# WHOIGit/ifcb_classifier

Hardware: AMD Instinct MI355X
Metric: train images/sec, inception_v3 299^2 IFCB ROIs (higher is better)
Workload: dtype bf16; 1 GPU; inception_v3 100-class bf16 TRAIN, batch 256 per GPU, synthetic u8 ROIs h,w~U{32..299} resized on-GPU to 299x299 (BASELINE.json configs[1]); global_batch=256, parallelism=dp1, program_lanes=4, IFCBK_LANES=4, weight_gradient_lanes=1, optimizer=adam lr=1e-3, loss=CE + 0.4*CE_aux, input_pipeline=preprocess then step on one stream

## Files before the change

ifcb_classifier_amd/csrc/conv_common.h:

```cpp
#pragma once
#include "common.h"

namespace {

struct ConvArgs {
    const void* x;
    const void* w;
    void* y;
    float* part;
    const float* ep_scale;
    const float* ep_shift;
    const void* ep_res;
    int ep_ldr, ep_relu;
    const void* bs_raw;
    const float *bs_mean, *bs_invstd, *bs_scale, *bs_shift;
    int bs_ld;
    const void* pad_;
    unsigned xbytes, wbytes;
    int H, W, C, ldx;
    int K, R, S;
    int P, Q, ldy;
    int ostr_h, ostr_w, base_h, base_w, ish, isw;
    int M, Kg;
    int accumulate;
    int seg_n, seg_end[4], seg_ld[4], seg_aff[4];
    void* seg_y[4];
    int PQ;
    int tilesN;
    int wKg, wSfull, w_rbase, w_sbase;
    int oH, oW, o_a, o_b;
    fastdiv_t fPQ, fQ;
    int tr;
    fastdiv_t fP;
    int dbg;
};

typedef const __attribute__((address_space(1))) void* gptr_t;
typedef __attribute__((address_space(3))) void* lptr_t;

template <class T> struct Mma;
template <> struct Mma<bf16_t> {
    typedef bf16x8_t frag_t;
    __device__ static __forceinline__ void run(const frag_t& a, const frag_t& b, f32x4_t& c) {
        c = __builtin_amdgcn_mfma_f32_16x16x32_bf16(a, b, c, 0, 0, 0);
    }
    __device__ static __forceinline__ void pack4(bf16_t* p, const f32x4_t& v) {
        uint2 u;
        u.x = pack2bf(v[0], v[1]);
        u.y = pack2bf(v[2], v[3]);
        *reinterpret_cast<uint2*>(p) = u;
    }
};
template <> struct Mma<float> {
    typedef f32x4_t frag_t;
    __device__ static __forceinline__ void run(const frag_t& a, const frag_t& b, f32x4_t& c) {
#pragma unroll
        for (int j = 0; j < 4; ++j) c = __builtin_amdgcn_mfma_f32_16x16x4f32(a[j], b[j], c, 0, 0, 0);
    }
    __device__ static __forceinline__ void pack4(float* p, const f32x4_t& v) { *reinterpret_cast<f32x4_t*>(p) = v; }
};

__device__ __forceinline__ void lds_dma16(__amdgpu_buffer_rsrc_t rs, lptr_t dst, unsigned voff, int soff) {
    __builtin_amdgcn_raw_ptr_buffer_load_lds(rs, dst, 16, voff, soff, 0, 0);
}

template <int N>
__device__ __forceinline__ void wait_vmcnt() {
    asm volatile("s_waitcnt vmcnt(%0)" ::"n"(N) : "memory");
}


template <class T, int BM, int BN, int NTHREADS, int MODE>
__device__ __forceinline__ void conv_epilogue_store(const ConvArgs& a, T* sC, float* sRed, const int t, const int lane, const int wave,
                                                    const int m0, const int n0, const int mtile) {
    constexpr bool BSTAT = MODE == 3;
    constexpr int ES = (int)sizeof(T);
    constexpr int CE = 16 / ES;
    constexpr int NW = NTHREADS / 64;
    constexpr int CPR = BN / CE;
    constexpr int CPRP = CPR <= 4 ? 4 : CPR <= 8 ? 8 : CPR <= 16 ? 16 : 32;
    constexpr int LDC = BN + CE;
    {
        constexpr int RPP = NTHREADS / CPRP;
        const int cc = t & (CPRP - 1);
        const int r0 = t / CPRP;
        const bool cvalid = (cc < CPR) && (n0 + cc * CE < a.K);
        typedef float f32x2_t __attribute__((ext_vector_type(2)));
        f32x2_t s1p[CE / 2], s2p[CE / 2];
#pragma unroll
        for (int j = 0; j < CE / 2; ++j) s1p[j] = s2p[j] = f32x2_t{0.f, 0.f};
        if (cvalid) {
            const int nn = n0 + cc * CE;
            float bmu[CE], bis[CE], bsc[CE], bsh[CE];
            if (BSTAT) {
#pragma unroll
                for (int j = 0; j < CE; ++j) {
                    bmu[j] = a.bs_mean[nn + j];
                    bis[j] = a.bs_invstd[nn + j];
                    bsc[j] = a.bs_scale[nn + j];
                    bsh[j] = a.bs_shift[nn + j];
                }
            }
            float sc[CE], sh[CE];
            if (a.ep_scale) {
#pragma unroll
                for (int j = 0; j < CE; ++j) {
                    sc[j] = a.ep_scale[nn + j];
                    sh[j] = a.ep_shift[nn + j];
                }
            }
            T* segbase = (T*)a.y + nn;
            int segld = a.ldy;
            bool seg_aff = true;
            if (MODE == 4) {
                int si = 0;
#pragma unroll
                for (int q = 0; q < 3; ++q)
                    if (q + 1 < a.seg_n && nn >= a.seg_end[q]) si = q + 1;
                segbase = (T*)a.seg_y[si] + (nn - (si ? a.seg_end[si - 1] : 0));
// ... 128 lines not shown
```

ifcb_classifier_amd/csrc/conv_igemm.hip:

```cpp
#include "conv_common.h"
#include <stdlib.h>

namespace {

template <class T, int NT, int WM, int NSTAGE, int MODE>
__global__ __launch_bounds__(128 * WM) void conv_igemm(ConvArgs a) {
    constexpr bool STRIDED = MODE == 1;
    constexpr int ES = (int)sizeof(T);
    constexpr int CE = 16 / ES;
    constexpr int BK = 128 / ES;
    typedef typename Mma<T>::frag_t frag_t;
    constexpr int NW = 2 * WM;
    constexpr int NTHREADS = 64 * NW;
    constexpr int BM = 64 * WM;
    constexpr int BN = 32 * NT;
    constexpr int JB = (NT * 4 + NW - 1) / NW;
    constexpr int G = 4 + JB;
    constexpr int D = NSTAGE - 1;
    constexpr int LDC = BN + CE;
    constexpr int STAGE = (BM + BN) * BK;
    constexpr int STAGE_BYTES = NSTAGE * STAGE * ES;
    constexpr int CT_BYTES = BM * LDC * ES + NW * BN * 2 * 4;
    constexpr int MAIN_BYTES = STAGE_BYTES > CT_BYTES ? STAGE_BYTES : CT_BYTES;
    constexpr int DUMMY_BYTES = (JB * NW > NT * 4) ? 1024 : 0;
    __shared__ __attribute__((aligned(16))) unsigned char smem[MAIN_BYTES + DUMMY_BYTES];
    T* sStage = reinterpret_cast<T*>(smem);
    T* sC = reinterpret_cast<T*>(smem);
    float* sRed = reinterpret_cast<float*>(smem + BM * LDC * ES);
    T* sDummy = reinterpret_cast<T*>(smem + MAIN_BYTES);

    const int t = threadIdx.x;
    const int lane = t & 63;
    const int wave = __builtin_amdgcn_readfirstlane(t >> 6);
    const int wm = wave >> 1, wn = wave & 1;
    const int bid = (int)xcd_remap(blockIdx.x, gridDim.x);
    const int mtile = bid / a.tilesN, ntile = bid - mtile * a.tilesN;
    const int m0 = mtile * BM, n0 = ntile * BN;

    const __amdgpu_buffer_rsrc_t rsA = __builtin_amdgcn_make_buffer_rsrc((void*)a.x, 0, a.xbytes, 0x00020000);
    const __amdgpu_buffer_rsrc_t rsB = __builtin_amdgcn_make_buffer_rsrc((void*)a.w, 0, a.wbytes, 0x00020000);
    constexpr unsigned OOB = 0x80000000u;
    const int lrow8 = lane >> 3;
    const int csrc = (lane & 7) ^ lrow8;
    int off0[4], bh[4], bw[4];
#pragma unroll
    for (int j = 0; j < 4; ++j) {
        int m = m0 + (wave * 4 + j) * 8 + lrow8;
        bool rv = m < a.M;
        int mm = rv ? m : 0;
        int n = (int)fdiv((uint32_t)mm, a.fPQ);
        int rem = mm - n * a.PQ;
        int p = (int)fdiv((uint32_t)rem, a.fQ);
        int q = rem - p * a.Q;
        bh[j] = rv ? p * a.ostr_h + a.base_h : -(1 << 24);
        bw[j] = q * a.ostr_w + a.base_w;
        off0[j] = STRIDED ? n * a.H * a.W * a.ldx : ((n * a.H + bh[j]) * a.W + bw[j]) * a.ldx;
    }
    int kc, kr, ks, tapoff;
    {
        kc = csrc * CE;
        kr = 0;
        ks = 0;
        while (kc >= a.C) {
            kc -= a.C;
            if (++ks == a.S) { ks = 0; ++kr; }
        }
        tapoff = (kr * a.W + ks) * a.ldx + kc;
    }
    int wk = MODE == 2 ? ((a.w_rbase + 2 * kr) * a.wSfull + a.w_sbase + 2 * ks) * a.C + kc : 0;
    unsigned woff[JB];
    bool gvalid[JB];
#pragma unroll
    for (int j = 0; j < JB; ++j) {
        int grp = j * NW + wave;
        gvalid[j] = grp < NT * 4;
        int n = n0 + grp * 8 + lrow8;
        woff[j] = (gvalid[j] && n < a.K) ? (MODE == 2 ? (unsigned)(n * a.wKg) : (unsigned)(n * a.Kg + csrc * CE)) * (unsigned)ES : OOB;
    }
    const int nk = (a.Kg + BK - 1) / BK;
    const int hmask = (1 << a.ish) - 1, wmask = (1 << a.isw) - 1;
    const int rowstep = a.W * a.ldx, colwrap = a.S * a.ldx;
    const int wrowskip = MODE == 2 ? (2 * a.wSfull - 2 * a.S) * a.C : 0;

    const bool plain = (MODE == 0 || MODE == 3 || MODE == 4) && a.R == 1 && a.S == 1 && a.base_h == 0 && a.base_w == 0;
    unsigned va[4];
#pragma unroll
    for (int j = 0; j < 4; ++j) va[j] = bh[j] >= 0 ? (unsigned)(off0[j] + csrc * CE) * (unsigned)ES : OOB;
    const bool ktail_ok = (nk - 1) * BK + csrc * CE < a.Kg;

#define ISSUE_TILE(kt, stage)                                                                              \
    {                                                                                                      \
        T* dstA = sStage + (stage) * STAGE;                                                                \
        T* dstB = dstA + BM * BK;                                                                          \
        if (plain) {                                                                                       \
            const bool cut = (kt) == nk - 1 && !ktail_ok;                                                  \
            _Pragma("unroll") for (int j = 0; j < 4; ++j)                                                  \
                lds_dma16(rsA, (lptr_t)(dstA + (wave * 4 + j) * 8 * BK), cut ? OOB : va[j], (kt) * 128);   \
        } else {                                                                                           \
            const bool kvalid = kr < a.R;                                                                  \
            _Pragma("unroll") for (int j = 0; j < 4; ++j) {                                                \
                int hr = bh[j] + kr, wr = bw[j] + ks;                                                      \
                unsigned voff;                                                                             \
                if (STRIDED) {                                                                             \
                    bool v = kvalid && hr >= 0 && wr >= 0 && ((hr & hmask) == 0) && ((wr & wmask) == 0);   \
                    int hi = hr >> a.ish, wi = wr >> a.isw;                                                \
                    v = v && hi < a.H && wi < a.W;                                                         \
                    voff = v ? (unsigned)(off0[j] + (hi * a.W + wi) * a.ldx + kc) * (unsigned)ES : OOB;    \
                } else {                                                                                   \
                    bool v = kvalid && (unsigned)hr < (unsigned)a.H && (unsigned)wr < (unsigned)a.W;       \
                    voff = v ? (unsigned)(off0[j] + tapoff) * (unsigned)ES : OOB;                          \
                }                                                                                          \
                __builtin_amdgcn_raw_ptr_buffer_load_lds(rsA, (lptr_t)(dstA + (wave * 4 + j) * 8 * BK), 16, voff, 0, 0, 0); \
            }                                                                                              \
        }                                                                                                  \
        if (MODE == 2) {                                                                                   \
            const bool kv2 = ((kt) * BK + csrc * CE) < a.Kg;                                               \
            _Pragma("unroll") for (int j = 0; j < JB; ++j) {                                               \
                unsigned voff = (kv2 && woff[j] != OOB) ? woff[j] + (unsigned)wk * (unsigned)ES : OOB;     \
// ... 5 lines not shown
            _Pragma("unroll") for (int j = 0; j < JB; ++j) {                                               \
                T* dst = gvalid[j] ? dstB + (j * NW + wave) * 8 * BK : sDummy;                             \
                lds_dma16(rsB, (lptr_t)dst, woff[j], (kt) * 128);                                          \
            }                                                                                              \
        }                                                                                                  \
        if (!plain) {                                                                                      \
            kc += BK;                                                                                      \
            tapoff += BK;                                                                                  \
            if (MODE == 2) wk += BK;                                                                       \
            while (kc >= a.C) {                                                                            \
                kc -= a.C;                                                                                 \
                tapoff += a.ldx - a.C;                                                                     \
                if (MODE == 2) wk += a.C;                       \
                if (++ks == a.S) { ks = 0; ++kr; tapoff += rowstep - colwrap; if (MODE == 2) wk += wrowskip; } \
            }                                                                                              \
        }                                                                                                  \
    }

    f32x4_t acc[NT][4];
#pragma unroll
    for (int i = 0; i < NT; ++i)
#pragma unroll
        for (int j = 0; j < 4; ++j) acc[i][j] = f32x4_t{0.f, 0.f, 0.f, 0.f};

#pragma unroll
    for (int d = 0; d < D; ++d)
        if (d < nk) ISSUE_TILE(d, d)

    const int frow = lane & 15, fchunk = lane >> 4;
    const T* fA[2];
    const T* fB[2];
#pragma unroll
    for (int kk = 0; kk < 2; ++kk) {
        const int ph = ((kk * 4 + fchunk) ^ (frow & 7)) * CE;
        fA[kk] = sStage + (wm * 64 + frow) * BK + ph;
        fB[kk] = sStage + BM * BK + (wn * (NT * 16) + frow) * BK + ph;
    }
    int stage = 0;
    int istage = D % NSTAGE;
    for (int kt = 0; kt < nk; ++kt) {
        const int newer = nk - 1 - kt < D - 1 ? nk - 1 - kt : D - 1;
        if (D >= 3 && newer >= 2) wait_vmcnt<2 * G>();
        else if (D >= 2 && newer >= 1) wait_vmcnt<G>();
        else wait_vmcnt<0>();
        __builtin_amdgcn_s_barrier();
        if (kt + D < nk) ISSUE_TILE(kt + D, istage)
        const int soff = stage * STAGE;
#pragma unroll
        for (int kk = 0; kk < 2; ++kk) {
            frag_t fa[4], fb[NT];
            const T* pa = fA[kk] + soff;
            const T* pb = fB[kk] + soff;
#pragma unroll
            for (int mt = 0; mt < 4; ++mt) fa[mt] = *reinterpret_cast<const frag_t*>(pa + mt * 16 * BK);
#pragma unroll
            for (int nt = 0; nt < NT; ++nt) fb[nt] = *reinterpret_cast<const frag_t*>(pb + nt * 16 * BK);
#pragma unroll
            for (int nt = 0; nt < NT; ++nt)
#pragma unroll
                for (int mt = 0; mt < 4; ++mt)
                    Mma<T>::run(fb[nt], fa[mt], acc[nt][mt]);
        }
        stage = stage + 1 == NSTAGE ? 0 : stage + 1;
        istage = istage + 1 == NSTAGE ? 0 : istage + 1;
    }
#undef ISSUE_TILE
    __syncthreads();

    {
        const int g = lane >> 4;
#pragma unroll
        for (int nt = 0; nt < NT; ++nt)
#pragma unroll
            for (int mt = 0; mt < 4; ++mt) {
                int m = wm * 64 + mt * 16 + frow;
                int n = wn * (NT * 16) + nt * 16 + 4 * g;
                Mma<T>::pack4(sC + m * LDC + n, acc[nt][mt]);
            }
    }
    __syncthreads();
    conv_epilogue_store<T, BM, BN, NTHREADS, MODE>(a, sC, sRed, t, lane, wave, m0, n0, mtile);
}

template <int NT>
__global__ __launch_bounds__(512) void conv_ws(ConvArgs a, int total_tiles) {
    typedef bf16_t T;
    constexpr int ES = 2, CE = 8, BK = 64, BM = 128, BN = 32 * NT, NSTAGE = 3;
    constexpr int STAGE = (BM + BN) * BK;
    constexpr int G = 4 + NT;
    __shared__ __attribute__((aligned(16))) unsigned char smem[NSTAGE * STAGE * ES];
    T* sStage = reinterpret_cast<T*>(smem);
    const int t = threadIdx.x, lane = t & 63;
    const int wave = __builtin_amdgcn_readfirstlane(t >> 6);
    const int b0 = (int)xcd_remap(blockIdx.x, gridDim.x);
    const int ngrid = (int)gridDim.x;
    const int ntl = (total_tiles - b0 + ngrid - 1) / ngrid;
    const int nk = (a.Kg + BK - 1) / BK;
    const int total_steps = ntl * nk;

    if (wave >= 4) {
        const int p = wave - 4;
        const __amdgpu_buffer_rsrc_t rsA = __builtin_amdgcn_make_buffer_rsrc((void*)a.x, 0, a.xbytes, 0x00020000);
        const __amdgpu_buffer_rsrc_t rsB = __builtin_amdgcn_make_buffer_rsrc((void*)a.w, 0, a.wbytes, 0x00020000);
        constexpr unsigned OOB = 0x80000000u;
        const int lrow8 = lane >> 3;
        const int csrc = (lane & 7) ^ lrow8;
        const bool plain = a.R == 1 && a.S == 1 && a.base_h == 0 && a.base_w == 0;
        const bool ktail_ok = (nk - 1) * BK + csrc * CE < a.Kg;
        const int rowstep = a.W * a.ldx, colwrap = a.S * a.ldx;
        int off0[4], bh[4], bw[4];
        unsigned va[4], woff[NT];
        int kc = 0, kr = 0, ks = 0, tapoff = 0, kt_issue = 0, r_issue = 0;
#define WS_SETUP_TILE(tile)                                                                                   \
        {                                                                                                     \
            const int mtile_ = (tile) / a.tilesN, ntile_ = (tile) - mtile_ * a.tilesN;                        \
            const int m0_ = mtile_ * BM, n0_ = ntile_ * BN;                                                   \
            _Pragma("unroll") for (int j = 0; j < 4; ++j) {                                                   \
                int m = m0_ + (p * 4 + j) * 8 + lrow8;                                                        \
                bool rv = m < a.M;                                                                            \
                int mm = rv ? m : 0;                                                                          \
                int n = (int)fdiv((uint32_t)mm, a.fPQ);                                                       \
                int rem = mm - n * a.PQ;                                                                      \
                int pp = (int)fdiv((uint32_t)rem, a.fQ);                                                      \
                int q = rem - pp * a.Q;                                                                       \
                bh[j] = rv ? pp * a.ostr_h + a.base_h : -(1 << 24);                                           \
                bw[j] = q * a.ostr_w + a.base_w;                                                              \
                off0[j] = ((n * a.H + bh[j]) * a.W + bw[j]) * a.ldx;                                          \
                va[j] = bh[j] >= 0 ? (unsigned)(off0[j] + csrc * CE) * (unsigned)ES : OOB;                    \
            }                                                                                                 \
            _Pragma("unroll") for (int j = 0; j < NT; ++j) {                                                  \
                int n = n0_ + (j * 4 + p) * 8 + lrow8;                                                        \
                woff[j] = n < a.K ? (unsigned)(n * a.Kg + csrc * CE) * (unsigned)ES : OOB;                    \
            }                                                                                                 \
            kc = csrc * CE; kr = 0; ks = 0;                                                                   \
            while (kc >= a.C) { kc -= a.C; if (++ks == a.S) { ks = 0; ++kr; } }                               \
            tapoff = (kr * a.W + ks) * a.ldx + kc;                                                            \
        }
#define WS_ISSUE(stage)                                                                                       \
        {                                                                                                     \
            if (kt_issue == 0) WS_SETUP_TILE(b0 + r_issue * ngrid)                                            \
            T* dstA = sStage + (stage) * STAGE;                                                               \
            T* dstB = dstA + BM * BK;                                                                         \
            if (plain) {                                                                                      \
                const bool cut = kt_issue == nk - 1 && !ktail_ok;                                             \
                _Pragma("unroll") for (int j = 0; j < 4; ++j)                                                 \
                    lds_dma16(rsA, (lptr_t)(dstA + (p * 4 + j) * 8 * BK), cut ? OOB : va[j], kt_issue * 128); \
            } else {                                                                                          \
                const bool kvalid = kr < a.R;                                                                 \
                _Pragma("unroll") for (int j = 0; j < 4; ++j) {                                               \
                    int hr = bh[j] + kr, wr = bw[j] + ks;                                                     \
                    bool v = kvalid && (unsigned)hr < (unsigned)a.H && (unsigned)wr < (unsigned)a.W;          \
                    unsigned voff = v ? (unsigned)(off0[j] + tapoff) * (unsigned)ES : OOB;                    \
                    __builtin_amdgcn_raw_ptr_buffer_load_lds(rsA, (lptr_t)(dstA + (p * 4 + j) * 8 * BK), 16, voff, 0, 0, 0); \
                }                                                                                             \
                kc += BK;                                                                                     \
                tapoff += BK;                                                                                 \
                while (kc >= a.C) {                                                                           \
                    kc -= a.C;                                                                                \
                    tapoff += a.ldx - a.C;                                                                    \
                    if (++ks == a.S) { ks = 0; ++kr; tapoff += rowstep - colwrap; }                           \
                }                                                                                             \
            }                                                                                                 \
            _Pragma("unroll") for (int j = 0; j < NT; ++j)                                                    \
                lds_dma16(rsB, (lptr_t)(dstB + (j * 4 + p) * 8 * BK), woff[j], kt_issue * 128);               \
            if (++kt_issue == nk) { kt_issue = 0; ++r_issue; }                                                \
        }
// ... 74 lines not shown
                    sc[j] = nv ? a.ep_scale[ncol + nt * 16 + j] : 0.f;
                    sh[j] = nv ? a.ep_shift[ncol + nt * 16 + j] : 0.f;
                }
            }
            f32x2_t s1[2] = {f32x2_t{0.f, 0.f}, f32x2_t{0.f, 0.f}}, s2[2] = {f32x2_t{0.f, 0.f}, f32x2_t{0.f, 0.f}};
#pragma unroll
            for (int mt = 0; mt < 4; ++mt) {
                f32x4_t v = acc[nt][mt];
                if (a.ep_scale) {
#pragma unroll
                    for (int j = 0; j < 4; ++j) {
                        v[j] = bf2f(f2bf(v[j])) * sc[j] + sh[j];
                        if (a.ep_relu) v[j] = fmaxf(v[j], 0.f);
                    }
                }
                uint2 u;
                u.x = pack2bf(v[0], v[1]);
                u.y = pack2bf(v[2], v[3]);
                if (mv[mt] && nv) *reinterpret_cast<uint2*>(row[mt] + nt * 16) = u;
                const f32x2_t lo = {__uint_as_float(u.x << 16), __uint_as_float(u.x & 0xffff0000u)};
                const f32x2_t hi = {__uint_as_float(u.y << 16), __uint_as_float(u.y & 0xffff0000u)};
                s1[0] += lo; s1[1] += hi;
                s2[0] += lo * lo; s2[1] += hi * hi;
            }
            if (a.part) {
#pragma unroll
                for (int off = 1; off < 16; off <<= 1)
#pragma unroll
                    for (int h = 0; h < 2; ++h)
#pragma unroll
                        for (int j = 0; j < 2; ++j) {
                            s1[h][j] += __shfl_xor(s1[h][j], off);
                            s2[h][j] += __shfl_xor(s2[h][j], off);
                        }
                if (frow == 0 && nv) {
                    float* prow = a.part + ((size_t)(mtile * 2 + wm) * 2) * a.K + ncol + nt * 16;
#pragma unroll
                    for (int j = 0; j < 4; ++j) {
                        prow[j] = s1[j >> 1][j & 1];
                        prow[a.K + j] = s2[j >> 1][j & 1];
                    }
                }
            }
        }
    }
}

int pick_nt(int K, int maxnt) {
    static int force = -1;
    if (force < 0) { const char* e = getenv("IFCBK_CONV_NT"); force = e ? atoi(e) : 0; }
    if (force > 0 && force <= maxnt) return force;
    int best = 1;
    long bestc = -1;
    for (int nt = 1; nt <= maxnt; ++nt) {
        int bn = 32 * nt;
        long c = (long)cdiv(K, bn) * (bn + 48);
        if (bestc < 0 || c < bestc || (c == bestc && nt > best)) { bestc = c; best = nt; }
    }
    return best;
}

int check_desc(ifcbk_ctx* ctx, const ifcbk_conv_desc* d, bool dgrad = false) {
    if (!d) IFCBK_FAIL(ctx, IFCBK_EINVAL, "conv: null desc");
    if (d->dtype != IFCBK_BF16 && d->dtype != IFCBK_F32) IFCBK_FAIL(ctx, IFCBK_EUNSUPPORTED, "conv: dtype must be bf16 or f32");
    const int ce = dtype_chunk(d->dtype), es = dtype_esize(d->dtype);
    if (d->C % ce || d->K % ce || d->ldx % ce || d->ldy % ce || d->C <= 0 || d->K <= 0)
        IFCBK_FAIL(ctx, IFCBK_EINVAL, "conv: C=%d K=%d ldx=%d ldy=%d must be positive multiples of %d", d->C, d->K, d->ldx, d->ldy, ce);
    if (d->stride_h < 1 || d->stride_w < 1 || (dgrad && (d->stride_h > 2 || d->stride_w > 2)))
        IFCBK_FAIL(ctx, IFCBK_EINVAL, "conv: stride must be >= 1 (1 or 2 for the input gradient)");
    int P = (d->H + 2 * d->pad_h - d->R) / d->stride_h + 1, Q = (d->W + 2 * d->pad_w - d->S) / d->stride_w + 1;
    if (P != d->P || Q != d->Q) IFCBK_FAIL(ctx, IFCBK_EINVAL, "conv: P,Q=%d,%d inconsistent (expect %d,%d)", d->P, d->Q, P, Q);
    if ((int64_t)d->N * d->P * d->Q * d->ldy * es >= (1ll << 31) || (int64_t)d->N * d->H * d->W * d->ldx * es >= (1ll << 31))
        IFCBK_FAIL(ctx, IFCBK_EINVAL, "conv: a tensor exceeds the 2 GiB buffer-descriptor window");
    return 0;
}

int pick_wm(int M, int K) {
    static int force = -1;
    if (force < 0) { const char* e = getenv("IFCBK_CONV_WM"); force = e ? atoi(e) : 0; }
    (void)M; (void)K;
    return force == 4 ? 4 : 2;
}

template <class T, int NT, int WM, int NSTAGE>
void launch(const ConvArgs& a, hipStream_t st) {
    int tilesM = cdiv(a.M, 64 * WM);
    dim3 grid((unsigned)(tilesM * a.tilesN)), block(128 * WM);
    if (a.seg_n) hipLaunchKernelGGL((conv_igemm<T, NT, WM, NSTAGE, 4>), grid, block, 0, st, a);
    else if (a.bs_raw) hipLaunchKernelGGL((conv_igemm<T, NT, WM, NSTAGE, 3>), grid, block, 0, st, a);
    else if (a.wKg) hipLaunchKernelGGL((conv_igemm<T, NT, WM, NSTAGE, 2>), grid, block, 0, st, a);
    else if (a.ish | a.isw) hipLaunchKernelGGL((conv_igemm<T, NT, WM, NSTAGE, 1>), grid, block, 0, st, a);
    else hipLaunchKernelGGL((conv_igemm<T, NT, WM, NSTAGE, 0>), grid, block, 0, st, a);
}

int ws_min_steps() {
    static int v = -1;
    if (v < 0) { const char* e = getenv("IFCBK_CONV_WS"); v = e ? atoi(e) : 4; }
    return v;
}
int num_cus();
int ws_max_tiles() {
    static int v = -1;
    if (v < 0) { const char* e = getenv("IFCBK_CONV_WS_TILES"); v = e ? atoi(e) : 2 * num_cus(); }
    return v;
}
bool ws_shape_ok(int dtype, int M, int K, int Kg) {
    const int ms = ws_min_steps();
    if (ms <= 0 || dtype != IFCBK_BF16 || pick_wm(M, K) != 2 || cdiv(Kg, 64) < ms) return false;
    const int nt = pick_nt(K, 6);
    return (int64_t)cdiv(M, 128) * cdiv(K, 32 * nt) <= ws_max_tiles();
}
int num_cus() {
    static int n = 0;
    if (!n) {
        int dev = 0;
        hipDeviceProp_t pr;
        if (hipGetDevice(&dev) == hipSuccess && hipGetDeviceProperties(&pr, dev) == hipSuccess) n = pr.multiProcessorCount;
        if (n <= 0) n = 256;
    }
    return n;
}

template <int NT>
void launch_ws(const ConvArgs& a, hipStream_t st) {
    const int total = cdiv(a.M, 128) * a.tilesN;
    const int grid = total < num_cus() ? total : num_cus();
    hipLaunchKernelGGL((conv_ws<NT>), dim3((unsigned)grid), dim3(512), 0, st, a, total);
}

bool big_ok(const ConvArgs& a) { return !a.wKg && !(a.ish | a.isw); }
bool pp3_ok(const ConvArgs& a) {
    return big_ok(a) && !a.seg_n && !a.bs_raw && !a.accumulate && !a.ep_res && (a.ep_scale == nullptr || a.part == nullptr);
}

int run(ifcbk_ctx* ctx, ConvArgs& a, int dtype, hipStream_t st) {
    const bool f32 = dtype == IFCBK_F32;
    if (!a.wKg && !(a.ish | a.isw) && a.ostr_h == 1 && a.ostr_w == 1 && !a.seg_n && !a.accumulate && !a.ep_res && a.PQ > 0) {
        const int N = a.M / a.PQ;
        if (ifcbk_conv_flat_rows(dtype, N, a.H, a.W, a.C, a.K, a.R, a.S, -a.base_h, -a.base_w, a.P, a.Q) > 0)
            return ifcbk_conv_flat_launch(ctx, &a, N, st);
    }
    if (big_ok(a) && a.ostr_h == 1 && a.ostr_w == 1 && !a.seg_n && a.PQ > 0) {
        const int N = a.M / a.PQ;
        if (ifcbk_conv_slab_plan(dtype, N, a.H, a.W, a.C, a.K, a.R, a.S, -a.base_h, -a.base_w, a.P, a.Q) > 0)
            return ifcbk_conv_slab_launch(ctx, &a, N, st);
    }
    if (pp3_ok(a) && ifcbk_conv_pp3_plan(dtype, a.M, a.K, a.Kg, a.ep_scale ? 1 : 0)) return ifcbk_conv_pp3_launch(ctx, &a, st);
    {
        int bmt = 0, btn = 0;
        if (big_ok(a) && ifcbk_conv_big_plan(dtype, a.M, a.K, a.Kg, &bmt, &btn)) return ifcbk_conv_big_launch(ctx, &a, bmt, btn, st);
    }
    int wm = f32 ? 2 : pick_wm(a.M, a.K);
    int nt = pick_nt(a.K, f32 ? 4 : (wm == 4 ? 5 : 6));
    a.tilesN = cdiv(a.K, 32 * nt);
    if ((int64_t)cdiv(a.M, 64 * wm) * a.tilesN >= (1ll << 31)) IFCBK_FAIL(ctx, IFCBK_EINVAL, "conv: grid too large");
    if (ws_shape_ok(dtype, a.M, a.K, a.Kg) && !a.seg_n && !a.bs_raw && !a.wKg && !(a.ish | a.isw) && !a.accumulate && !a.ep_res) {
        switch (nt) {
            case 1: launch_ws<1>(a, st); break;
            case 2: launch_ws<2>(a, st); break;
            case 3: launch_ws<3>(a, st); break;
            case 4: launch_ws<4>(a, st); break;
            case 5: launch_ws<5>(a, st); break;
            default: launch_ws<6>(a, st); break;
        }
        IFCBK_LAUNCH_CHECK(ctx, "conv_ws");
        return 0;
    }
    if (f32) {
        switch (nt) {
            case 1: launch<float, 1, 2, 2>(a, st); break;
            case 2: launch<float, 2, 2, 2>(a, st); break;
            case 3: launch<float, 3, 2, 2>(a, st); break;
            default: launch<float, 4, 2, 2>(a, st); break;
        }
    } else if (wm == 4) {
        switch (nt) {
            case 1: launch<bf16_t, 1, 4, 3>(a, st); break;
            case 2: launch<bf16_t, 2, 4, 3>(a, st); break;
            case 3: launch<bf16_t, 3, 4, 3>(a, st); break;
            case 4: launch<bf16_t, 4, 4, 3>(a, st); break;
            default: launch<bf16_t, 5, 4, 3>(a, st); break;
        }
    } else {
        switch (nt) {
            case 1: launch<bf16_t, 1, 2, 2>(a, st); break;
            case 2: launch<bf16_t, 2, 2, 2>(a, st); break;
            case 3: launch<bf16_t, 3, 2, 2>(a, st); break;
            case 4: launch<bf16_t, 4, 2, 2>(a, st); break;
            case 5: launch<bf16_t, 5, 2, 2>(a, st); break;
            default: launch<bf16_t, 6, 2, 2>(a, st); break;
        }
    }
    IFCBK_LAUNCH_CHECK(ctx, "conv_igemm");
    return 0;
}

}

int ifcbk_num_cus() { return num_cus(); }

int ifcbk_conv_fwd_nt(int K, int M) { return pick_nt(K, pick_wm(M, K) == 4 ? 5 : 6); }

int ifcbk_conv_fwd_wm(int M, int K) { return pick_wm(M, K); }

bool ifcbk_conv_ws_shape(int dtype, int M, int K, int Kg) { return ws_shape_ok(dtype, M, K, Kg); }

static bool fwd_rows(const ifcbk_conv_desc* d) {
    return ifcbk_conv_rows_ok(d->dtype, d->C, d->K, d->R, d->S, d->stride_h, d->stride_w, d->pad_h, d->pad_w, d->Q);
}

extern "C" int ifcbk_conv2d_fwd_mblocks(const ifcbk_conv_desc* d) {
    if (fwd_rows(d)) return ifcbk_conv_rows_blocks(d->N, d->P);
    int M = d->N * d->P * d->Q;
    if (d->stride_h == 1 && d->stride_w == 1)
        if (int fs = ifcbk_conv_flat_rows(d->dtype, d->N, d->H, d->W, d->C, d->K, d->R, d->S, d->pad_h, d->pad_w, d->P, d->Q)) return fs;
    if (d->stride_h == 1 && d->stride_w == 1)
        if (int smt = ifcbk_conv_slab_plan(d->dtype, d->N, d->H, d->W, d->C, d->K, d->R, d->S, d->pad_h, d->pad_w, d->P, d->Q)) return cdiv(M, 32 * smt);
    if (ifcbk_conv_pp3_plan(d->dtype, M, d->K, d->R * d->S * d->C, 0)) return 2 * cdiv(M, 256);
    {
        int bmt = 0, btn = 0;
        if (ifcbk_conv_big_plan(d->dtype, M, d->K, d->R * d->S * d->C, &bmt, &btn)) return cdiv(M, 32 * bmt);
    }
    if (ws_shape_ok(d->dtype, M, d->K, d->R * d->S * d->C)) return 2 * cdiv(M, 128);
    return cdiv(M, 64 * pick_wm(M, d->K));
}

struct FwdSegs { int n, end[4], ld[4], aff[4]; void* y[4]; };
static int conv_fwd_impl(ifcbk_ctx* ctx, const ifcbk_conv_desc* d, const void* x, const void* w, void* y, float* bn_part,
                         const float* scale, const float* shift, const void* residual, int ldr, int relu, void* stream,
                         const FwdSegs* seg = nullptr);

extern "C" int ifcbk_conv2d_fwd_affine_segments(ifcbk_ctx* ctx, const ifcbk_conv_desc* d, const void* x, const void* w, int nseg,
                                                void* const* ys, const int32_t* ldys, const int32_t* ksegs, const int32_t* affine,
                                                const float* scale, const float* shift, void* stream) {
    if (!d || nseg < 1 || nseg > 4 || !ys || !ldys || !ksegs || !affine || !scale || !shift)
        IFCBK_FAIL(ctx, IFCBK_EINVAL, "conv2d_fwd_affine_segments: bad args");
    FwdSegs sg;
    sg.n = nseg;
    int end = 0;
    const int ce = dtype_chunk(d->dtype);
    for (int q = 0; q < 4; ++q) {
        const bool live = q < nseg;
        if (live) {
            if (!ys[q] || ksegs[q] <= 0 || ksegs[q] % ce || ldys[q] % ce)
                IFCBK_FAIL(ctx, IFCBK_EINVAL, "conv2d_fwd_affine_segments: segment %d: null / size not a multiple of %d", q, ce);
            end += ksegs[q];
        }
        sg.end[q] = end; sg.ld[q] = live ? ldys[q] : 0; sg.aff[q] = live ? affine[q] : 0; sg.y[q] = live ? ys[q] : nullptr;
    }
    if (end != d->K) IFCBK_FAIL(ctx, IFCBK_EINVAL, "conv2d_fwd_affine_segments: segment sizes sum to %d, K=%d", end, d->K);
    return conv_fwd_impl(ctx, d, x, w, ys[0], nullptr, scale, shift, nullptr, 0, 1, stream, &sg);
}

extern "C" int ifcbk_conv2d_fwd(ifcbk_ctx* ctx, const ifcbk_conv_desc* d, const void* x, const void* w, void* y,
                                float* bn_part, void* stream) {
    return conv_fwd_impl(ctx, d, x, w, y, bn_part, nullptr, nullptr, nullptr, 0, 0, stream);
}

extern "C" int ifcbk_conv2d_fwd_affine(ifcbk_ctx* ctx, const ifcbk_conv_desc* d, const void* x, const void* w, void* y,
                                       const float* scale, const float* shift, const void* residual, int ldr, int relu,
                                       void* stream) {
    if (!scale || !shift) IFCBK_FAIL(ctx, IFCBK_EINVAL, "conv2d_fwd_affine: scale/shift required");
    return conv_fwd_impl(ctx, d, x, w, y, nullptr, scale, shift, residual, ldr, relu, stream);
}

extern "C" int ifcbk_conv2d_fwd_affine_maxpool_ok(const ifcbk_conv_desc* d) {
    return d && ifcbk_conv_rows_pool_ok(d->dtype, d->C, d->K, d->R, d->S, d->stride_h, d->stride_w, d->pad_h, d->pad_w, d->P, d->Q) ? 1 : 0;
}

extern "C" int ifcbk_conv2d_fwd_affine_maxpool(ifcbk_ctx* ctx, const ifcbk_conv_desc* d, const void* x, const void* w, void* y_pooled,
                                               int ldp, const float* scale, const float* shift, int relu, void* stream) {
    if (!ifcbk_conv2d_fwd_affine_maxpool_ok(d)) IFCBK_FAIL(ctx, IFCBK_EUNSUPPORTED, "conv2d_fwd_affine_maxpool: not served by the row-streaming kernel");
    if (!x || !w || !y_pooled || !scale || !shift || ldp < d->K || ldp % 8) IFCBK_FAIL(ctx, IFCBK_EINVAL, "conv2d_fwd_affine_maxpool: bad operand");
// ... 56 lines not shown
    a.seg_n = seg ? seg->n : 0;
    for (int q = 0; q < 4; ++q) {
        a.seg_end[q] = seg ? seg->end[q] : 0; a.seg_ld[q] = seg ? seg->ld[q] : 0; a.seg_aff[q] = seg ? seg->aff[q] : 0;
        a.seg_y[q] = seg ? seg->y[q] : nullptr;
    }
    const int es = dtype_esize(d->dtype);
    a.xbytes = (unsigned)((int64_t)d->N * d->H * d->W * d->ldx * es); a.wbytes = (unsigned)((int64_t)d->K * d->R * d->S * d->C * es);
    a.H = d->H; a.W = d->W; a.C = d->C; a.ldx = d->ldx;
    a.K = d->K; a.R = d->R; a.S = d->S;
    a.P = d->P; a.Q = d->Q; a.ldy = d->ldy;
    a.ostr_h = d->stride_h; a.ostr_w = d->stride_w; a.base_h = -d->pad_h; a.base_w = -d->pad_w;
    a.ish = 0; a.isw = 0;
    a.wKg = 0; a.wSfull = 0; a.w_rbase = 0; a.w_sbase = 0; a.oH = 0; a.oW = 0; a.o_a = 0; a.o_b = 0;
    a.M = d->N * d->P * d->Q; a.Kg = d->R * d->S * d->C; a.accumulate = 0; a.PQ = d->P * d->Q;
    a.fPQ = make_fastdiv(a.PQ); a.fQ = make_fastdiv(a.Q);
    return run(ctx, a, d->dtype, (hipStream_t)stream);
}

struct BnStatArgs {
    const void* raw;
    int ld;
    const float *mean, *invstd, *scale, *shift;
    float* part;
};

static bool dgrad_bnstat_ok(const ifcbk_conv_desc* d) {
    if (d->stride_h != 1 || d->stride_w != 1) return false;
    return !ifcbk_conv_rows_ok(d->dtype, d->K, d->C, d->R, d->S, d->stride_h, d->stride_w, 2 - d->pad_h, 2 - d->pad_w, d->W);
}

static int dgrad_impl(ifcbk_ctx* ctx, const ifcbk_conv_desc* d, const void* dy, const void* wT, void* dx, int accumulate,
                      const BnStatArgs* bs, void* stream);

extern "C" int ifcbk_conv2d_dgrad(ifcbk_ctx* ctx, const ifcbk_conv_desc* d, const void* dy, const void* wT, void* dx,
                                  int accumulate, void* stream) {
    return dgrad_impl(ctx, d, dy, wT, dx, accumulate, nullptr, stream);
}

extern "C" int ifcbk_conv2d_dgrad_bnstat_mblocks(const ifcbk_conv_desc* d) {
    if (!d || !dgrad_bnstat_ok(d)) return 0;
    int M = d->N * d->H * d->W;
    if (int fs = ifcbk_conv_flat_rows(d->dtype, d->N, d->P, d->Q, d->K, d->C, d->R, d->S, d->R - 1 - d->pad_h, d->S - 1 - d->pad_w, d->H, d->W)) return fs;
    if (int smt = ifcbk_conv_slab_plan(d->dtype, d->N, d->P, d->Q, d->K, d->C, d->R, d->S, d->R - 1 - d->pad_h, d->S - 1 - d->pad_w, d->H, d->W)) return cdiv(M, 32 * smt);
    {
        int bmt = 0, btn = 0;
        if (ifcbk_conv_big_plan(d->dtype, M, d->C, d->R * d->S * d->K, &bmt, &btn)) return cdiv(M, 32 * bmt);
    }
    return cdiv(M, 64 * pick_wm(M, d->C));
}

extern "C" int ifcbk_conv2d_dgrad_bnstat(ifcbk_ctx* ctx, const ifcbk_conv_desc* d, const void* dy, const void* wT, void* dx,
                                         const void* prev_raw, int prev_ld, const float* prev_mean, const float* prev_invstd,
                                         const float* prev_scale, const float* prev_shift, float* part, void* stream) {
    if (!d || !dgrad_bnstat_ok(d)) IFCBK_FAIL(ctx, IFCBK_EUNSUPPORTED, "conv2d_dgrad_bnstat: stride-1 implicit-GEMM input gradients only");
    if (!prev_raw || !prev_mean || !prev_invstd || !prev_scale || !prev_shift || !part)
        IFCBK_FAIL(ctx, IFCBK_EINVAL, "conv2d_dgrad_bnstat: null operand");
    BnStatArgs bs = {prev_raw, prev_ld, prev_mean, prev_invstd, prev_scale, prev_shift, part};
    return dgrad_impl(ctx, d, dy, wT, dx, 0, &bs, stream);
}

static int dgrad_impl(ifcbk_ctx* ctx, const ifcbk_conv_desc* d, const void* dy, const void* wT, void* dx, int accumulate,
                      const BnStatArgs* bs, void* stream) {
    if (int e = check_desc(ctx, d, true)) return e;
    if (!bs && !accumulate && ifcbk_conv_rows_ok(d->dtype, d->K, d->C, d->R, d->S, d->stride_h, d->stride_w, 2 - d->pad_h, 2 - d->pad_w, d->W))
        return ifcbk_conv_rows_launch(ctx, d->K, d->C, d->N, d->P, d->Q, d->ldy, d->H, d->W, d->ldx, 2 - d->pad_h, 2 - d->pad_w, dy,
                                      wT, dx, nullptr, nullptr, nullptr, 0, (hipStream_t)stream);
    ConvArgs a;
    a.dbg = 0; a.tr = 0; a.fP = make_fastdiv(1);
    a.ep_scale = nullptr; a.ep_shift = nullptr; a.ep_res = nullptr; a.ep_ldr = 0; a.ep_relu = 0;
    a.x = dy; a.w = wT; a.y = dx; a.part = bs ? bs->part : nullptr;
    a.seg_n = 0;
    a.bs_raw = bs ? bs->raw : nullptr; a.bs_ld = bs ? bs->ld : 0;
    a.bs_mean = bs ? bs->mean : nullptr; a.bs_invstd = bs ? bs->invstd : nullptr;
    a.bs_scale = bs ? bs->scale : nullptr; a.bs_shift = bs ? bs->shift : nullptr;
    const int es = dtype_esize(d->dtype);
    a.xbytes = (unsigned)((int64_t)d->N * d->P * d->Q * d->ldy * es); a.wbytes = (unsigned)((int64_t)d->K * d->R * d->S * d->C * es);
    a.H = d->P; a.W = d->Q; a.C = d->K; a.ldx = d->ldy;
    a.K = d->C; a.R = d->R; a.S = d->S;
    a.P = d->H; a.Q = d->W; a.ldy = d->ldx;
    a.ostr_h = 1; a.ostr_w = 1;
    a.wKg = 0; a.wSfull = 0; a.w_rbase = 0; a.w_sbase = 0; a.oH = 0; a.oW = 0; a.o_a = 0; a.o_b = 0;
    a.accumulate = accumulate;
    if (d->stride_h == 2 && d->stride_w == 2 && d->R >= 2 && d->S >= 2 && d->H >= 2 && d->W >= 2) {
        for (int pa = 0; pa < 2; ++pa)
            for (int pb = 0; pb < 2; ++pb) {
                const int r0 = (pa + d->pad_h) & 1, s0 = (pb + d->pad_w) & 1;
                const int nU = (d->R - r0 + 1) / 2, nV = (d->S - s0 + 1) / 2;
                const int Hc = (d->H - pa + 1) / 2, Wc = (d->W - pb + 1) / 2;
                ConvArgs c = a;
                c.R = nU; c.S = nV;
                c.P = Hc; c.Q = Wc;
                c.base_h = (pa + d->pad_h - r0) / 2 - (nU - 1);
                c.base_w = (pb + d->pad_w - s0) / 2 - (nV - 1);
                c.ish = 0; c.isw = 0;
                c.wKg = d->R * d->S * d->K; c.wSfull = d->S;
                c.w_rbase = d->R - 1 - r0 - 2 * (nU - 1); c.w_sbase = d->S - 1 - s0 - 2 * (nV - 1);
                c.oH = d->H; c.oW = d->W; c.o_a = pa; c.o_b = pb;
                c.M = d->N * Hc * Wc; c.Kg = nU * nV * d->K; c.PQ = Hc * Wc;
                c.fPQ = make_fastdiv(c.PQ); c.fQ = make_fastdiv(c.Q);
                if (int e = run(ctx, c, d->dtype, (hipStream_t)stream)) return e;
            }
        return 0;
    }
    a.base_h = -(d->R - 1 - d->pad_h); a.base_w = -(d->S - 1 - d->pad_w);
    a.ish = d->stride_h == 2 ? 1 : 0; a.isw = d->stride_w == 2 ? 1 : 0;
    a.M = d->N * d->H * d->W; a.Kg = d->R * d->S * d->K; a.PQ = d->H * d->W;
    a.fPQ = make_fastdiv(a.PQ); a.fQ = make_fastdiv(a.Q);
    return run(ctx, a, d->dtype, (hipStream_t)stream);
}
```

ifcb_classifier_amd/engine.py:

```python
import ctypes as C
import math
import os

import torch

from . import _lib
from ._lib import Op, ConvDesc, BnDesc, PoolDesc, HeadDesc, RoiDesc


_DISPATCH_SWITCHES = ('IFCBK_CONV_PP3', 'IFCBK_CONV_PP3_GRID', 'IFCBK_WGRAD_LANE', 'IFCBK_WGRAD_GROUP', 'IFCBK_WGRAD_GROUP_MINKH', 'IFCBK_CONV_BIG', 'IFCBK_CONV_SLAB', 'IFCBK_CONV_BIG_MT', 'IFCBK_CONV_BIG_TN', 'IFCBK_CONV_FLAT', 'IFCBK_CONV_NT',
                      'IFCBK_CONV_WM', 'IFCBK_CONV_WS', 'IFCBK_CONV_WS_TILES', 'IFCBK_CONV_ROWS', 'IFCBK_WGRAD_PP',
                      'IFCBK_WGRAD_PP_KH', 'IFCBK_WGRAD_COLS', 'IFCBK_WGRAD_STEM', 'IFCBK_WGRAD_ROUNDS', 'IFCBK_WGRAD_FLAT',
                      'IFCBK_BN_BWD_ROWS')


def _dispatch_env():
    return tuple(os.environ.get(k) for k in _DISPATCH_SWITCHES)


def dtype_is_bf16(eng):
    return eng.dtype == 'bf16'


def _vp(t, byte_off=0):
    return None if t is None else C.c_void_p(t.data_ptr() + byte_off)


class OpList:

    def __init__(self):
        self.ops = []
        self.tags = []
        self.meta = []

    def add(self, kind, tag, p=(), i=(), f=(), flags=0, conv=None, bn=None, pool=None, head=None, lane=0, reads=None,
            writes=None):
        o = Op()
        o.kind, o.flags = kind, flags
        self.meta.append((lane, reads, writes))
        for k, v in enumerate(p):
            o.p[k] = v if (v is None or isinstance(v, int)) else v.value
        for k, v in enumerate(i):
            o.i[k] = int(v)
        for k, v in enumerate(f):
            o.f[k] = float(v)
        if conv is not None:
            o.u.conv = conv
        elif bn is not None:
            o.u.bn = bn
        elif pool is not None:
            o.u.pool = pool
        elif head is not None:
            o.u.head = head
        self.ops.append(o)
        self.tags.append(tag)
        return o

    def extend(self, other):
        self.ops.extend(other.ops)
        self.tags.extend(other.tags)
        self.meta.extend(other.meta)

    def slice(self, b0, b1):
        sub = OpList()
        sub.ops, sub.tags, sub.meta = self.ops[b0:b1], self.tags[b0:b1], self.meta[b0:b1]
        return sub

    def freeze(self):
        arr = (Op * len(self.ops))(*self.ops)
        for k, (lane, wait) in enumerate(schedule_lanes(self.meta)):
            arr[k].flags = (arr[k].flags & 0xff) | (lane << 8) | (wait << 12)
        return arr


def _overlap(a, b):
    return a[:-2] == b[:-2] and a[-2] < b[-1] and b[-2] < a[-1]


def schedule_lanes(meta):
    NL = 8
    count = [0] * NL
    synced = [[0] * NL for _ in range(NL)]
    table = {}
    star = ('*', 0, 1)
    out = []
    for lane, reads, writes in meta:
        if reads is None and writes is None:
            lane, reads, writes = 0, [star], [star]
        else:
            reads, writes = list(reads or ()) + [star], list(writes or ())
        deps = set()
        for r in reads:
            for res, (w, _rd) in table.items():
                if w is not None and _overlap(r, res):
                    deps.add(w)
        for wres in writes:
# ... 1529 lines not shown
```

Baseline: 12190 images/s.

## Launch all four stride-2 dgrad parity classes in one grid

The stride-2 input-gradient convolution used to issue four separate kernel launches, one per output parity class. They are now merged into a single launch whose blocks index a per-class table, with the classes sorted so the longest-Kg class comes first. This is meant to cut launch overhead and the tail-idle time between small back-to-back grids. Each block pays for a small class lookup and a copy of the table into kernel arguments. An environment switch restores the old per-class launches.

Result: no change. 12230 images/s, median of 6 (+0.4%).

```diff
diff --git a/ifcb_classifier_amd/csrc/conv_common.h b/ifcb_classifier_amd/csrc/conv_common.h
--- a/ifcb_classifier_amd/csrc/conv_common.h
+++ b/ifcb_classifier_amd/csrc/conv_common.h
@@ -35,6 +35,16 @@
     int dbg;
 };
 
+struct S2Class {
+    int R, S, P, Q, M, Kg, PQ;
+    int base_h, base_w, w_rbase, w_sbase, o_a, o_b;
+    int first, nblk;
+    fastdiv_t fPQ, fQ;
+};
+struct S2Grid {
+    S2Class c[4];
+};
+
 typedef const __attribute__((address_space(1))) void* gptr_t;
 typedef __attribute__((address_space(3))) void* lptr_t;
 
diff --git a/ifcb_classifier_amd/csrc/conv_igemm.hip b/ifcb_classifier_amd/csrc/conv_igemm.hip
--- a/ifcb_classifier_amd/csrc/conv_igemm.hip
+++ b/ifcb_classifier_amd/csrc/conv_igemm.hip
@@ -1,10 +1,11 @@
 #include "conv_common.h"
+#include <limits.h>
 #include <stdlib.h>
 
 namespace {
 
 template <class T, int NT, int WM, int NSTAGE, int MODE>
-__global__ __launch_bounds__(128 * WM) void conv_igemm(ConvArgs a) {
+__device__ __forceinline__ void conv_igemm_block(const ConvArgs a, const unsigned blk, const unsigned nblk) {
     constexpr bool STRIDED = MODE == 1;
     constexpr int ES = (int)sizeof(T);
     constexpr int CE = 16 / ES;
@@ -33,7 +34,7 @@
     const int lane = t & 63;
     const int wave = __builtin_amdgcn_readfirstlane(t >> 6);
     const int wm = wave >> 1, wn = wave & 1;
-    const int bid = (int)xcd_remap(blockIdx.x, gridDim.x);
+    const int bid = (int)xcd_remap(blk, nblk);
     const int mtile = bid / a.tilesN, ntile = bid - mtile * a.tilesN;
     const int m0 = mtile * BM, n0 = ntile * BN;
 
@@ -205,6 +206,25 @@
     conv_epilogue_store<T, BM, BN, NTHREADS, MODE>(a, sC, sRed, t, lane, wave, m0, n0, mtile);
 }
 
+template <class T, int NT, int WM, int NSTAGE, int MODE>
+__global__ __launch_bounds__(128 * WM) void conv_igemm(ConvArgs a) {
+    conv_igemm_block<T, NT, WM, NSTAGE, MODE>(a, blockIdx.x, gridDim.x);
+}
+
+template <class T, int NT, int WM, int NSTAGE, int MODE>
+__global__ __launch_bounds__(128 * WM) void conv_igemm(ConvArgs a, S2Grid g) {
+    static_assert(MODE == 2, "the class table belongs to the stride-2 input gradient");
+    const int b = (int)blockIdx.x;
+    const int ci = (b >= g.c[1].first ? 1 : 0) + (b >= g.c[2].first ? 1 : 0) + (b >= g.c[3].first ? 1 : 0);
+    const S2Class& c = g.c[ci];
+    const int local = b - c.first;
+    if (local >= c.nblk) return;
+    a.R = c.R; a.S = c.S; a.P = c.P; a.Q = c.Q; a.M = c.M; a.Kg = c.Kg; a.PQ = c.PQ;
+    a.base_h = c.base_h; a.base_w = c.base_w; a.w_rbase = c.w_rbase; a.w_sbase = c.w_sbase; a.o_a = c.o_a; a.o_b = c.o_b;
+    a.fPQ = c.fPQ; a.fQ = c.fQ;
+    conv_igemm_block<T, NT, WM, NSTAGE, 2>(a, (unsigned)local, (unsigned)c.nblk);
+}
+
 template <int NT>
 __global__ __launch_bounds__(512) void conv_ws(ConvArgs a, int total_tiles) {
     typedef bf16_t T;
@@ -445,13 +465,32 @@
     return force == 4 ? 4 : 2;
 }
 
+int64_t s2_layout(S2Grid* s2, int ncls, int bm, int tilesN) {
+    int64_t total = 0;
+    for (int i = 0; i < 4; ++i) {
+        S2Class& c = s2->c[i];
+        if (i >= ncls) { c = s2->c[0]; c.first = INT_MAX; c.nblk = 0; continue; }
+        total = (total + 7) & ~(int64_t)7;
+        const int64_t n = (int64_t)cdiv(c.M, bm) * tilesN;
+        c.first = (int)(total < INT_MAX ? total : INT_MAX);
+        c.nblk = (int)(n < INT_MAX ? n : INT_MAX);
+        total += n;
+    }
+    return total;
+}
+
 template <class T, int NT, int WM, int NSTAGE>
-void launch(const ConvArgs& a, hipStream_t st) {
+void launch(const ConvArgs& a, hipStream_t st, const S2Grid* s2, int ncls) {
+    if (s2) {
+        S2Grid g = *s2;
+        dim3 grid((unsigned)s2_layout(&g, ncls, 64 * WM, a.tilesN)), block(128 * WM);
+        hipLaunchKernelGGL((conv_igemm<T, NT, WM, NSTAGE, 2>), grid, block, 0, st, a, g);
+        return;
+    }
     int tilesM = cdiv(a.M, 64 * WM);
     dim3 grid((unsigned)(tilesM * a.tilesN)), block(128 * WM);
     if (a.seg_n) hipLaunchKernelGGL((conv_igemm<T, NT, WM, NSTAGE, 4>), grid, block, 0, st, a);
     else if (a.bs_raw) hipLaunchKernelGGL((conv_igemm<T, NT, WM, NSTAGE, 3>), grid, block, 0, st, a);
-    else if (a.wKg) hipLaunchKernelGGL((conv_igemm<T, NT, WM, NSTAGE, 2>), grid, block, 0, st, a);
     else if (a.ish | a.isw) hipLaunchKernelGGL((conv_igemm<T, NT, WM, NSTAGE, 1>), grid, block, 0, st, a);
     else hipLaunchKernelGGL((conv_igemm<T, NT, WM, NSTAGE, 0>), grid, block, 0, st, a);
 }
@@ -496,8 +535,9 @@
     return big_ok(a) && !a.seg_n && !a.bs_raw && !a.accumulate && !a.ep_res && (a.ep_scale == nullptr || a.part == nullptr);
 }
 
-int run(ifcbk_ctx* ctx, ConvArgs& a, int dtype, hipStream_t st) {
+int run(ifcbk_ctx* ctx, ConvArgs& a, int dtype, hipStream_t st, const S2Grid* s2 = nullptr, int ncls = 0) {
     const bool f32 = dtype == IFCBK_F32;
+    if ((a.wKg != 0) != (s2 != nullptr)) IFCBK_FAIL(ctx, IFCBK_EINVAL, "conv: a parity-class launch needs its class table");
     if (!a.wKg && !(a.ish | a.isw) && a.ostr_h == 1 && a.ostr_w == 1 && !a.seg_n && !a.accumulate && !a.ep_res && a.PQ > 0) {
         const int N = a.M / a.PQ;
         if (ifcbk_conv_flat_rows(dtype, N, a.H, a.W, a.C, a.K, a.R, a.S, -a.base_h, -a.base_w, a.P, a.Q) > 0)
@@ -517,6 +557,10 @@
     int nt = pick_nt(a.K, f32 ? 4 : (wm == 4 ? 5 : 6));
     a.tilesN = cdiv(a.K, 32 * nt);
     if ((int64_t)cdiv(a.M, 64 * wm) * a.tilesN >= (1ll << 31)) IFCBK_FAIL(ctx, IFCBK_EINVAL, "conv: grid too large");
+    if (s2) {
+        S2Grid g = *s2;
+        if (s2_layout(&g, ncls, 64 * wm, a.tilesN) >= (1ll << 31)) IFCBK_FAIL(ctx, IFCBK_EINVAL, "conv: grid too large");
+    }
     if (ws_shape_ok(dtype, a.M, a.K, a.Kg) && !a.seg_n && !a.bs_raw && !a.wKg && !(a.ish | a.isw) && !a.accumulate && !a.ep_res) {
         switch (nt) {
             case 1: launch_ws<1>(a, st); break;
@@ -531,27 +575,27 @@
     }
     if (f32) {
         switch (nt) {
-            case 1: launch<float, 1, 2, 2>(a, st); break;
-            case 2: launch<float, 2, 2, 2>(a, st); break;
-            case 3: launch<float, 3, 2, 2>(a, st); break;
-            default: launch<float, 4, 2, 2>(a, st); break;
+            case 1: launch<float, 1, 2, 2>(a, st, s2, ncls); break;
+            case 2: launch<float, 2, 2, 2>(a, st, s2, ncls); break;
+            case 3: launch<float, 3, 2, 2>(a, st, s2, ncls); break;
+            default: launch<float, 4, 2, 2>(a, st, s2, ncls); break;
         }
     } else if (wm == 4) {
         switch (nt) {
-            case 1: launch<bf16_t, 1, 4, 3>(a, st); break;
-            case 2: launch<bf16_t, 2, 4, 3>(a, st); break;
-            case 3: launch<bf16_t, 3, 4, 3>(a, st); break;
-            case 4: launch<bf16_t, 4, 4, 3>(a, st); break;
-            default: launch<bf16_t, 5, 4, 3>(a, st); break;
+            case 1: launch<bf16_t, 1, 4, 3>(a, st, s2, ncls); break;
+            case 2: launch<bf16_t, 2, 4, 3>(a, st, s2, ncls); break;
+            case 3: launch<bf16_t, 3, 4, 3>(a, st, s2, ncls); break;
+            case 4: launch<bf16_t, 4, 4, 3>(a, st, s2, ncls); break;
+            default: launch<bf16_t, 5, 4, 3>(a, st, s2, ncls); break;
         }
     } else {
         switch (nt) {
-            case 1: launch<bf16_t, 1, 2, 2>(a, st); break;
-            case 2: launch<bf16_t, 2, 2, 2>(a, st); break;
-            case 3: launch<bf16_t, 3, 2, 2>(a, st); break;
-            case 4: launch<bf16_t, 4, 2, 2>(a, st); break;
-            case 5: launch<bf16_t, 5, 2, 2>(a, st); break;
-            default: launch<bf16_t, 6, 2, 2>(a, st); break;
+            case 1: launch<bf16_t, 1, 2, 2>(a, st, s2, ncls); break;
+            case 2: launch<bf16_t, 2, 2, 2>(a, st, s2, ncls); break;
+            case 3: launch<bf16_t, 3, 2, 2>(a, st, s2, ncls); break;
+            case 4: launch<bf16_t, 4, 2, 2>(a, st, s2, ncls); break;
+            case 5: launch<bf16_t, 5, 2, 2>(a, st, s2, ncls); break;
+            default: launch<bf16_t, 6, 2, 2>(a, st, s2, ncls); break;
         }
     }
     IFCBK_LAUNCH_CHECK(ctx, "conv_igemm");
@@ -774,12 +818,16 @@
     a.wKg = 0; a.wSfull = 0; a.w_rbase = 0; a.w_sbase = 0; a.oH = 0; a.oW = 0; a.o_a = 0; a.o_b = 0;
     a.accumulate = accumulate;
     if (d->stride_h == 2 && d->stride_w == 2 && d->R >= 2 && d->S >= 2 && d->H >= 2 && d->W >= 2) {
+        const char* env = getenv("IFCBK_DGRAD_S2_GRID");
+        const bool one_grid = !env || atoi(env) != 0;
+        ConvArgs cls[4];
         for (int pa = 0; pa < 2; ++pa)
             for (int pb = 0; pb < 2; ++pb) {
                 const int r0 = (pa + d->pad_h) & 1, s0 = (pb + d->pad_w) & 1;
                 const int nU = (d->R - r0 + 1) / 2, nV = (d->S - s0 + 1) / 2;
                 const int Hc = (d->H - pa + 1) / 2, Wc = (d->W - pb + 1) / 2;
-                ConvArgs c = a;
+                ConvArgs& c = cls[pa * 2 + pb];
+                c = a;
                 c.R = nU; c.S = nV;
                 c.P = Hc; c.Q = Wc;
                 c.base_h = (pa + d->pad_h - r0) / 2 - (nU - 1);
@@ -790,9 +838,28 @@
                 c.oH = d->H; c.oW = d->W; c.o_a = pa; c.o_b = pb;
                 c.M = d->N * Hc * Wc; c.Kg = nU * nV * d->K; c.PQ = Hc * Wc;
                 c.fPQ = make_fastdiv(c.PQ); c.fQ = make_fastdiv(c.Q);
-                if (int e = run(ctx, c, d->dtype, (hipStream_t)stream)) return e;
             }
-        return 0;
+        auto class_of = [](const ConvArgs& c) {
+            S2Class s;
+            s.R = c.R; s.S = c.S; s.P = c.P; s.Q = c.Q; s.M = c.M; s.Kg = c.Kg; s.PQ = c.PQ;
+            s.base_h = c.base_h; s.base_w = c.base_w; s.w_rbase = c.w_rbase; s.w_sbase = c.w_sbase; s.o_a = c.o_a; s.o_b = c.o_b;
+            s.first = 0; s.nblk = 0;
+            s.fPQ = c.fPQ; s.fQ = c.fQ;
+            return s;
+        };
+        S2Grid g;
+        if (!one_grid) {
+            for (int i = 0; i < 4; ++i) {
+                g.c[0] = class_of(cls[i]);
+                if (int e = run(ctx, cls[i], d->dtype, (hipStream_t)stream, &g, 1)) return e;
+            }
+            return 0;
+        }
+        int order[4] = {0, 1, 2, 3};
+        for (int i = 1; i < 4; ++i)
+            for (int j = i; j > 0 && cls[order[j]].Kg > cls[order[j - 1]].Kg; --j) { const int t = order[j]; order[j] = order[j - 1]; order[j - 1] = t; }
+        for (int i = 0; i < 4; ++i) g.c[i] = class_of(cls[order[i]]);
+        return run(ctx, cls[order[0]], d->dtype, (hipStream_t)stream, &g, 4);
     }
     a.base_h = -(d->R - 1 - d->pad_h); a.base_w = -(d->S - 1 - d->pad_w);
     a.ish = d->stride_h == 2 ? 1 : 0; a.isw = d->stride_w == 2 ? 1 : 0;
diff --git a/ifcb_classifier_amd/engine.py b/ifcb_classifier_amd/engine.py
--- a/ifcb_classifier_amd/engine.py
+++ b/ifcb_classifier_amd/engine.py
@@ -11,7 +11,7 @@
 _DISPATCH_SWITCHES = ('IFCBK_CONV_PP3', 'IFCBK_CONV_PP3_GRID', 'IFCBK_WGRAD_LANE', 'IFCBK_WGRAD_GROUP', 'IFCBK_WGRAD_GROUP_MINKH', 'IFCBK_CONV_BIG', 'IFCBK_CONV_SLAB', 'IFCBK_CONV_BIG_MT', 'IFCBK_CONV_BIG_TN', 'IFCBK_CONV_FLAT', 'IFCBK_CONV_NT',
                       'IFCBK_CONV_WM', 'IFCBK_CONV_WS', 'IFCBK_CONV_WS_TILES', 'IFCBK_CONV_ROWS', 'IFCBK_WGRAD_PP',
                       'IFCBK_WGRAD_PP_KH', 'IFCBK_WGRAD_COLS', 'IFCBK_WGRAD_STEM', 'IFCBK_WGRAD_ROUNDS', 'IFCBK_WGRAD_FLAT',
-                      'IFCBK_BN_BWD_ROWS')
+                      'IFCBK_BN_BWD_ROWS', 'IFCBK_DGRAD_S2_GRID')
 
 
 def _dispatch_env():
```
